# cbouilla/spasm

Hardware: AMD Instinct MI355X
Metric: rows eliminated/sec (sparse Schur complement, mod 42013) (higher is better)
Workload: dtype i32 sums of i16 x i16 products

## Files before the change

spasm_amd/csrc/backsolve.hip:

```cpp
#include <algorithm>
#include <cinttypes>
#include <type_traits>
#include <thread>
#include <vector>

#include "device_types.h"
#include "field_dev.h"
#include "sgn_dev.h"

namespace sh {

int usable_cpus();

namespace {

constexpr int BS_RING = 768;
constexpr int BS_NEARCAP = 1024;
constexpr int BS_PASSCAP = 80;
constexpr int BS_PASSROWS = 32;
constexpr uint32_t BS_NONE = 0xFFFFFFFFu;

template <typename T> T *dalloc(int64_t count)
{
	return static_cast<T *>(sh::big_alloc((size_t) (count > 0 ? count : 1) * sizeof(T)));
}

template <typename T> void upload(T *dst, const std::vector<T> &src, hipStream_t s)
{
	if (!src.empty())
		sh::h2d(dst, src.data(), src.size() * sizeof(T), s);
}

struct BsArgs {
	void *R;
	int64_t ldR;
	int nchunks;
	const BsChunk *chunk;
	const int *chunk_extra;
	const uint4 *ptab;
	const uint2 *near;
	const uint4 *far_head;
	const uint64_t *far_rp;
	const uint2 *far;
	const uint64_t *np_rp;
	const uint2 *np;
	const int *np_row;
	int plain;
	int sparse_init;
	int r;
	unsigned long long *prof;
	int sgn;
	MontDev F;
	SgnDev G;
};

template <bool PACKED> struct Word {
	static constexpr int CPL = PACKED ? 2 : 1;
	using Elem = typename std::conditional<PACKED, uint16_t, uint32_t>::type;
};

template <bool PACKED, bool PLAIN> __device__ __forceinline__ uint32_t w_submul(uint32_t x, uint32_t v, uint32_t y, const MontDev &F, uint32_t bm)
{
	auto small = [&](uint32_t xe, uint32_t ve) -> uint32_t {
		const uint32_t t = __umul24(ve, y);
		const uint32_t q = __umulhi(t, bm);
		uint32_t rem = t - __umul24(q, F.p);
		rem = (rem >= F.p) ? rem - F.p : rem;
		rem = (rem >= F.p) ? rem - F.p : rem;
		return (xe >= rem) ? xe - rem : xe + F.p - rem;
	};
	if constexpr (PACKED) {
		static_assert(PLAIN, "packed entries only exist for p < 2^16");
		return small(x & 0xFFFFu, v & 0xFFFFu) | (small(x >> 16, v >> 16) << 16);
	} else if constexpr (PLAIN) {
		return small(x, v);
	} else {
		return submod(x, montmul(v, y, F), F);
	}
}

template <typename T> __global__ __launch_bounds__(256) void bs_init_kernel(BsArgs b)
{
// ... 38 lines not shown
}

template <int HI, bool FIRST> __device__ __forceinline__ void sgn_mad_half(uint32_t w, uint32_t c2, int &lo, int &hi)
{
	if constexpr (FIRST) {
		static_assert(HI == 0, "the first term takes the low coefficient");
		asm("v_mad_i32_i16 %0, %1, %2, 0" : "=v"(lo) : "v"(w), "v"(c2));
		asm("v_mad_i32_i16 %0, %1, %2, 0 op_sel:[1,0,0,0]" : "=v"(hi) : "v"(w), "v"(c2));
	} else if constexpr (HI == 0) {
		asm("v_mad_i32_i16 %0, %1, %2, %0" : "+v"(lo) : "v"(w), "v"(c2));
		asm("v_mad_i32_i16 %0, %1, %2, %0 op_sel:[1,0,0,0]" : "+v"(hi) : "v"(w), "v"(c2));
	} else {
		asm("v_mad_i32_i16 %0, %1, %2, %0 op_sel:[0,1,0,0]" : "+v"(lo) : "v"(w), "v"(c2));
		asm("v_mad_i32_i16 %0, %1, %2, %0 op_sel:[1,1,0,0]" : "+v"(hi) : "v"(w), "v"(c2));
	}
}

__host__ __device__ __forceinline__ uint4 bs_pass_empty(uint32_t spare_off)
{
	return uint4{spare_off, spare_off | (spare_off << 16), 0u, 0u};
}

template <int HI> __device__ __forceinline__ uint32_t bs_ring_at(uint32_t packed, uint32_t base)
{
	uint32_t a;
	if constexpr (HI == 0)
		asm("v_mad_u32_u16 %0, %1, 4, %2" : "=v"(a) : "v"(packed), "v"(base));
	else
		asm("v_mad_u32_u16 %0, %1, 4, %2 op_sel:[1,0,0,0]" : "=v"(a) : "v"(packed), "v"(base));
	return a;
}
using bs_lds_word = __attribute__((address_space(3))) uint32_t;

template <bool PACKED, int LPR, int NW, int RING = BS_RING, int PASSROWS = BS_PASSROWS, int PASSCAP = BS_PASSCAP> struct BsGeom {
	static constexpr int RING_ = RING, PASSROWS_ = PASSROWS, PASSCAP_ = PASSCAP;
	static constexpr int THREADS = 64 * NW;
	static constexpr int RS = 64 / LPR;
	static constexpr int CW = LPR * Word<PACKED>::CPL;
	static constexpr int ROWS_PER_ITER = RS * NW;
	static constexpr int ITERS = RING / ROWS_PER_ITER;
	static constexpr int UNR = (NW >= 8 && ITERS <= 24) ? ITERS : (ITERS % 12 == 0) ? 12 : 8;
	static constexpr int LANES_USED = RS * LPR;
	static_assert(RING % ROWS_PER_ITER == 0 && ITERS % UNR == 0, "phase A is unrolled in passes of UNR rows");
	static constexpr int N_NEAR = (BS_NEARCAP + THREADS - 1) / THREADS;
	static constexpr int N_ROW = (RING + THREADS - 1) / THREADS;
	static constexpr int N_PTAB = (PASSCAP * PASSROWS + THREADS - 1) / THREADS;
	static constexpr size_t FH_BYTES = (size_t) RING * sizeof(uint4);
	static constexpr size_t PTAB_BYTES = (size_t) PASSCAP * PASSROWS * sizeof(uint4);
	static constexpr int RSTR = LPR + 1;
	static constexpr size_t LDS_BYTES = FH_BYTES + PTAB_BYTES + (size_t) BS_NEARCAP * sizeof(uint2) + (size_t) (RING + 1) * RSTR * 4;
};

template <bool PACKED, bool PLAIN, int LPR, int NW, bool SGN = false, int RING = BS_RING, int PASSROWS = BS_PASSROWS, int PASSCAP = BS_PASSCAP, int WGS_PER_CU = 1>
__global__ __launch_bounds__(64 * NW, WGS_PER_CU) void backsolve_kernel(BsArgs b)
{
	static_assert(!SGN || (PACKED && PLAIN), "signed entries are packed 16-bit entries");
	const uint32_t bm = PLAIN ? (uint32_t) (0x100000000ull / b.F.p) : 0u;
	const SgnDev G = b.G;
	using Geo = BsGeom<PACKED, LPR, NW, RING, PASSROWS, PASSCAP>;
	using Elem = typename Word<PACKED>::Elem;
	extern __shared__ __attribute__((aligned(16))) unsigned char bs_lds[];
	uint4 *fh = reinterpret_cast<uint4 *>(bs_lds);
	uint4 *ptab = reinterpret_cast<uint4 *>(bs_lds + Geo::FH_BYTES);
	uint2 *near = reinterpret_cast<uint2 *>(bs_lds + Geo::FH_BYTES + Geo::PTAB_BYTES);
	uint32_t *ring = reinterpret_cast<uint32_t *>(near + BS_NEARCAP);
	const int tid = threadIdx.x;
	const int lane = tid & 63, wave = tid >> 6;
	auto lds_barrier = [&]() { asm volatile("s_waitcnt lgkmcnt(0)\n\ts_barrier" ::: "memory"); };
	const int rs = lane / LPR, wl = lane % LPR;
	constexpr int RSTR = Geo::RSTR;
	constexpr uint32_t SPARE = (uint32_t) (RING * RSTR);
	constexpr int WPW = LPR / NW, RSB = 64 / WPW;
	static_assert(WPW >= 1 && LPR % NW == 0 && 64 % WPW == 0, "every wave takes the same number of words of a row through phase B");
	static_assert(PASSROWS % RSB == 0, "a pass is a whole number of wave instructions");
	const MontDev F = b.F;
	const int64_t ldw = b.ldR / Word<PACKED>::CPL;
	uint32_t *Rs = static_cast<uint32_t *>(b.R) + (int64_t) blockIdx.x * LPR + wl;
	const uint32_t ldw256 = (uint32_t) (ldw >> 8);
	auto at_off = [&](uint32_t off) -> uint32_t * { return Rs + ((uint64_t) off << 8); };
	const int slot0 = wave * Geo::RS + rs;
	const uint32_t slot0_off = (uint32_t) slot0 * ldw256;
	const uint32_t iter_off = (uint32_t) Geo::ROWS_PER_ITER * ldw256;
	const bool lane_ok = lane < Geo::LANES_USED && (int64_t) blockIdx.x * LPR + wl < ldw;
	const int col_lo = blockIdx.x * Geo::CW;

	RegFile<uint2, Geo::N_NEAR> m_near;
	RegFile<uint4, Geo::N_ROW> m_fh;
	RegFile<uint4, Geo::N_PTAB> m_ptab;
	auto load_meta = [&](const BsChunk &c) {
		bs_static_for<0, Geo::N_NEAR>([&](auto qq) {
			constexpr int q = decltype(qq)::value;
			const int t = tid + q * Geo::THREADS;
			const uint2 v = b.near[(t < c.nnear) ? c.near0 + t : 0];
			m_near.template at<q>() = (t < c.nnear) ? v : uint2{0u, 0u};
		});
		bs_static_for<0, Geo::N_ROW>([&](auto qq) {
			constexpr int q = decltype(qq)::value;
			const int t = tid + q * Geo::THREADS;
			const uint4 v = b.far_head[(t < c.hi - c.lo) ? c.lo + t : 0];
			m_fh.template at<q>() = (t < c.hi - c.lo) ? v : bs_head<PLAIN>(BS_NONE, 0u, BS_NONE, 0u);
		});
		int tid_m = tid;
		asm volatile("" : "+v"(tid_m));
		bs_static_for<0, Geo::N_PTAB>([&](auto qq) {
			constexpr int q = decltype(qq)::value;
			const int t = tid_m + q * Geo::THREADS;
			const uint4 v = b.ptab[(t < c.npass * PASSROWS) ? (int64_t) c.pass0 * PASSROWS + t : 0];
			m_ptab.template at<q>() = (t < c.npass * PASSROWS) ? v : bs_pass_empty(SPARE);
		});
	};
	auto store_meta = [&]() {
		bs_static_for<0, Geo::N_NEAR>([&](auto qq) {
			constexpr int q = decltype(qq)::value;
			if (tid + q * Geo::THREADS < BS_NEARCAP)
				near[tid + q * Geo::THREADS] = m_near.template at<q>();
		});
		bs_static_for<0, Geo::N_ROW>([&](auto qq) {
// ... 12 lines not shown
	asm volatile("v_mov_b32 %0, 0" : "=v"(vzero));
	uint4 raw_a = uint4{0u, 0u, 0u, 0u}, raw_b = uint4{0u, 0u, 0u, 0u};
	auto fetch_chunk = [&](int k) {
		const uint4 *src = reinterpret_cast<const uint4 *>(b.chunk + k) + vzero;
		raw_a = src[0];
		raw_b = src[1];
	};
	auto fetched_chunk = [&]() {
		BsChunk c;
		c.lo = __builtin_amdgcn_readfirstlane((int) raw_a.x);
		c.hi = __builtin_amdgcn_readfirstlane((int) raw_a.y);
		c.pass0 = __builtin_amdgcn_readfirstlane((int) raw_a.z);
		c.npass = (unsigned short) __builtin_amdgcn_readfirstlane((int) (raw_a.w & 0xFFFFu));
		c.nord = (unsigned short) __builtin_amdgcn_readfirstlane((int) (raw_a.w >> 16));
		c.near0 = __builtin_amdgcn_readfirstlane((int) raw_b.x);
		c.nnear = __builtin_amdgcn_readfirstlane((int) raw_b.y);
		c.np0 = __builtin_amdgcn_readfirstlane((int) raw_b.z);
		c.npn = __builtin_amdgcn_readfirstlane((int) raw_b.w);
		return c;
	};
	BsChunk ch_next{};
	if (b.nchunks > 0) {
		fetch_chunk(0);
		ch_next = fetched_chunk();
		load_meta(ch_next);
		store_meta();
	}
	if (b.nchunks > 1)
		fetch_chunk(1);
	__syncthreads();

	unsigned long long pt[8] = {0, 0, 0, 0, 0, 0, 0, 0};
	unsigned long long t_last = 0;
	const bool profiling = b.prof != nullptr && blockIdx.x == 0 && tid == 0;
	auto tick = [&](int q) {
		if (profiling) {
			const unsigned long long now = __builtin_readcyclecounter();
			pt[q] += now - t_last;
			t_last = now;
		}
	};
	if (profiling)
		t_last = __builtin_readcyclecounter();
	for (int k = 0; k < b.nchunks; k++) {
		const BsChunk ch = ch_next;
		const int nrows = ch.hi - ch.lo;
		uint2 c_np = uint2{0u, 0u};
		int c_np_row = 0;
		if (b.sparse_init) {
			const int cnt = ch.npn & 0x7FFFFFFF;
			c_np = b.np[(tid < cnt) ? ch.np0 + tid : 0];
			c_np_row = b.np_row[(tid < cnt) ? ch.np0 + tid : 0];
		}
		if (k + 1 < b.nchunks) {
			ch_next = fetched_chunk();
			load_meta(ch_next);
		}
		if (k + 2 < b.nchunks)
			fetch_chunk(k + 2);
		tick(0);

		const uint32_t lo_off = (uint32_t) ch.lo * ldw256;
		auto phase_a = [&](auto sparse_tag) {
			constexpr bool SPARSE = decltype(sparse_tag)::value;
			for (int pass = 0; pass < Geo::ITERS / Geo::UNR; pass++) {
				if (pass * Geo::UNR * Geo::ROWS_PER_ITER >= nrows)
					break;
				constexpr bool KEEP = SPARSE && (PLAIN || NW < 16);
				uint32_t acc[SPARSE ? 1 : Geo::UNR], v0[Geo::UNR], v1[Geo::UNR], c0[KEEP ? Geo::UNR : 1], c1[(KEEP && !PLAIN) ? Geo::UNR : 1];
				uint32_t own_off = lo_off + (uint32_t) (pass * Geo::UNR) * iter_off + slot0_off;
				asm volatile("" : "+v"(own_off));
#pragma unroll
				for (int u = 0; u < Geo::UNR; u++) {
					const int s = (pass * Geo::UNR + u) * Geo::ROWS_PER_ITER + slot0;
					const bool ok = s < nrows && lane_ok;
					const uint4 h = fh[ok ? s : 0];
					const uint32_t a0 = h.x, a1 = PLAIN ? h.y : h.z;
					if constexpr (KEEP) {
						c0[u] = PLAIN ? h.z : h.y;
						if constexpr (!PLAIN)
							c1[u] = h.w;
					}
					if constexpr (!SPARSE) {
						acc[u] = ok ? *at_off(own_off) : 0u;
						own_off += iter_off;
					}
					if constexpr (LPR <= 16 && 64 % LPR == 0) {
						v0[u] = *at_off((ok && a0 != BS_NONE) ? a0 : lo_off);
						v1[u] = *at_off((ok && a1 != BS_NONE) ? a1 : lo_off);
					} else {
						v0[u] = (ok && a0 != BS_NONE) ? *at_off(a0) : 0u;
						v1[u] = (ok && a1 != BS_NONE) ? *at_off(a1) : 0u;
					}
				}
#pragma unroll
				for (int u = 0; u < Geo::UNR; u++) {
					const int s = (pass * Geo::UNR + u) * Geo::ROWS_PER_ITER + slot0;
					uint32_t x = SPARSE ? 0u : acc[u];
					uint32_t k0, k1;
					if constexpr (KEEP) {
						k0 = c0[u];
						k1 = PLAIN ? 0u : c1[u];
					} else if constexpr (PLAIN) {
						k0 = fh[s].z;
						k1 = 0u;
					} else {
						const uint4 h = fh[s];
						k0 = h.y;
						k1 = h.w;
					}
					if constexpr (SGN) {
						int lo, hi;
						if constexpr (SPARSE) {
							sgn_mad_half<0, true>(v0[u], k0, lo, hi);
						} else {
							sgn_unpack(x, lo, hi);
							sgn_mad_half<0, false>(v0[u], k0, lo, hi);
						}
						sgn_mad_half<1, false>(v1[u], k0, lo, hi);
						x = sgn_pack(sgn_reduce(lo, G), sgn_reduce(hi, G));
					} else {
						if constexpr (PLAIN) {
							k1 = k0 >> 16;
							k0 &= 0xFFFFu;
						}
						if (k0 != 0u)
							x = w_submul<PACKED, PLAIN>(x, v0[u], k0, F, bm);
						if (k1 != 0u)
							x = w_submul<PACKED, PLAIN>(x, v1[u], k1, F, bm);
					}
					if (s < nrows && lane_ok)
						ring[s * RSTR + wl] = x;
				}
			}
		};
		if (b.sparse_init)
			phase_a(std::true_type{});
		else
			phase_a(std::false_type{});
		lds_barrier();
		tick(1);
		if (b.sparse_init) {
			const int np_count = ch.npn & 0x7FFFFFFF;
			auto put = [&](const uint2 en, int row) {
				const int cc = (int) en.x - col_lo;
				if (cc >= 0 && cc < Geo::CW) {
					Elem *at = reinterpret_cast<Elem *>(ring) + (row - ch.lo) * (RSTR * Word<PACKED>::CPL) + cc;
					if constexpr (SGN) {
						*at = (Elem) (uint16_t) (int16_t) sgn_canonical((int) (int16_t) *at + sgn_from_residue(en.y, G), G);
					} else {
						const uint32_t v = PLAIN ? en.y : montmul(en.y, 1u, F);
						uint32_t sum = (uint32_t) *at + v;
						if (sum < v || sum >= F.p)
							sum -= F.p;
						*at = (Elem) sum;
					}
				}
			};
			if (tid < np_count)
				put(c_np, c_np_row);
			for (int e = Geo::THREADS + tid; e < np_count; e += Geo::THREADS)
				put(b.np[ch.np0 + e], b.np_row[ch.np0 + e]);
			lds_barrier();
		}
		tick(2);
		if (ch.npn < 0) {
			for (int s = slot0; s < nrows; s += Geo::ROWS_PER_ITER) {
				const int c = ch.lo + s;
				const uint64_t e0 = b.far_rp[c], e1 = b.far_rp[c + 1];
				if (e0 == e1 || !lane_ok)
					continue;
				uint32_t x = ring[s * RSTR + wl];
				if constexpr (SGN) {
					int lo, hi;
					sgn_unpack(x, lo, hi);
					for (uint64_t e = e0; e < e1; e += 4) {
#pragma unroll
						for (int t = 0; t < 4; t++) {
							const uint2 en = (e + t < e1) ? b.far[e + t] : uint2{0u, 0u};
							sgn_mad((e + t < e1) ? *at_off(en.x) : 0u, (int) en.y, lo, hi);
						}
						lo = sgn_reduce(lo, G);
						hi = sgn_reduce(hi, G);
					}
					x = sgn_pack(lo, hi);
				} else {
					for (uint64_t e = e0; e < e1; e++) {
						const uint2 en = b.far[e];
						x = w_submul<PACKED, PLAIN>(x, *at_off(en.x), en.y, F, bm);
					}
				}
				ring[s * RSTR + wl] = x;
			}
			lds_barrier();
		}

		tick(3);
		{
			constexpr int IPP = PASSROWS / RSB;
			const int niter = ch.npass * IPP;
			int tid_b = tid;
			asm volatile("" : "+v"(tid_b));
			const int rsb = (tid_b & 63) / WPW, wlb = (tid_b >> 6) * WPW + (tid_b & 63) % WPW;
			const uint4 *pe = ptab + rsb;
			const uint32_t wlb_at = (uint32_t) (uintptr_t) (bs_lds_word *) (ring + wlb);
			auto word = [&](uint32_t at) -> bs_lds_word & { return *reinterpret_cast<bs_lds_word *>((uintptr_t) at); };
			auto ordinary = [&](const uint4 e) {
				const uint32_t at_x = bs_ring_at<0>(e.x, wlb_at), at_0 = bs_ring_at<0>(e.y, wlb_at), at_1 = bs_ring_at<1>(e.y, wlb_at);
				if constexpr (SGN) {
					const uint32_t x0 = word(at_x), v0 = word(at_0), v1 = word(at_1);
					int lo, hi;
					sgn_unpack(x0, lo, hi);
					sgn_mad_half<0, false>(v0, e.z, lo, hi);
					sgn_mad_half<1, false>(v1, e.z, lo, hi);
					word(at_x) = sgn_pack(sgn_reduce(lo, G), sgn_reduce(hi, G));
				} else {
					const uint32_t c0 = PLAIN ? (e.z & 0xFFFFu) : e.z, c1 = PLAIN ? (e.z >> 16) : e.w;
					if (c0 != 0u) {
						uint32_t x = w_submul<PACKED, PLAIN>(word(at_x), word(at_0), c0, F, bm);
						if (c1 != 0u)
							x = w_submul<PACKED, PLAIN>(x, word(at_1), c1, F, bm);
						word(at_x) = x;
					}
				}
			};
// ... 33 lines not shown
			uint4 e = pe[0];
			int it = 0, run = ch.nord * IPP;
			while (it < niter) {
				const int stop = min(it + run, niter);
				for (; it + 1 < stop; it += 2) {
					const uint4 e_odd = pe[(it + 1) * RSB];
					ordinary(e);
					e = pe[(it + 2) * RSB];
					ordinary(e_odd);
				}
				if (it < stop) {
					const uint4 e_next = pe[(it + 1) * RSB];
					ordinary(e);
					e = e_next;
					it += 1;
				}
				if (it < niter) {
					run = __builtin_amdgcn_readfirstlane((int) (e.y >> 16)) * IPP;
					for (int q = 0; q < IPP; q++, it++) {
						const uint4 e_next = pe[(it + 1) * RSB];
						long_row(e);
						e = e_next;
					}
				}
			}
		}
		lds_barrier();
		tick(4);

		{
			uint32_t off = lo_off + slot0_off;
			asm volatile("" : "+v"(off));
			for (int s = slot0; s < nrows; s += Geo::ROWS_PER_ITER, off += iter_off)
				if (lane_ok)
					*at_off(off) = ring[s * RSTR + wl];
		}
		__syncthreads();
		tick(5);
		if (k + 1 < b.nchunks)
			store_meta();
		__syncthreads();
		tick(6);
	}
	if (profiling)
		for (int q = 0; q < 8; q++)
			b.prof[q] = pt[q];
}

constexpr int AP_LIST = 64;
constexpr int AP_TU = 4;

struct ApplyArgs {
	SchurArgs a;
	const void *R;
	int64_t ldR;
	const int *col;
	int r;
	int Smpad;
	int seg_words;
	int waves;
	size_t wave_bytes;
	uint32_t *dense_out;
	int64_t ldS;
	int direct;
	unsigned long long *status;
	int *ticket;
	int ntickets;
	int64_t *Sp;
	int *Sj;
	int *Sx;
// ... 252 lines not shown
						out_x[wpos + before] = to_balanced(v0, F);
					}
					if (v1 != 0) {
						const int64_t dst = wpos + before + (v0 != 0 ? 1 : 0);
						out_j[dst] = a.q[c0 + 1];
						out_x[dst] = to_balanced(v1, F);
					}
					wpos += __popcll(m0) + __popcll(m1);
				} else {
					const uint64_t mk = __ballot(w != 0);
					if (w != 0) {
						const int64_t dst = wpos + __popcll(mk & below);
						out_j[dst] = a.q[t0 + lane];
						out_x[dst] = to_balanced(w, F);
					}
					wpos += __popcll(mk);
				}
			}
		}
		if (lane == 0 && !d.direct) {
			if (fits) {
				a.row_off[k] = off | (1LL << 62);
				a.row_len[k] = count;
			} else {
				atomicOr(&a.ctr[CTR_STATUS], 1);
				a.row_len[k] = -1;
			}
		}
		st_done += fits ? 1 : 0;
	}
	apply_statistics(a, lane, st_input, st_piv, st_done, lost);
}

template <bool DEEP>
__device__ __forceinline__ int s16_reduce_segment(const ApplyArgs &d, const MontDev &F, const SgnDev &G, int64_t lo, int64_t hi, int w0, int nwords,
                                                  uint2 *plist, uint32_t *xw, int lane, bool first_seg, unsigned long long &st_piv)
{
	short *xe = reinterpret_cast<short *>(xw);
	const uint32_t *R = static_cast<const uint32_t *>(d.R);
	const uint32_t ldw256 = (uint32_t) (d.ldR / 2 / 256);
	for (int t = lane; t < nwords; t += 64)
		xw[t] = 0;
	int npl = 0;
	int count = -1;
	for (int64_t base = lo;; base += 64) {
		bool piv = false;
		uint32_t cid = 0;
		int bal = 0;
		if (base + lane < hi) {
			cid = (uint32_t) d.col[d.a.Aj[base + lane]];
			bal = sgn_from_residue(reduce_sum(from_balanced(d.a.Ax[base + lane], F), F), G);
			if (cid >= (uint32_t) d.r) {
				const uint32_t t = cid - (uint32_t) d.r - 2u * (uint32_t) w0;
				if (t < 2u * (uint32_t) nwords)
					xe[t] = (short) sgn_canonical((int) xe[t] + bal, G);
			} else {
				piv = bal != 0;
			}
		}
		const uint64_t mk = __ballot(piv);
		if (piv)
			plist[npl + __popcll(mk & ((1ull << lane) - 1ull))] = uint2{cid * ldw256, (uint32_t) (-bal)};
		npl += __popcll(mk);
		st_piv += first_seg ? (unsigned long long) __popcll(mk) : 0ull;
		const bool last = base + 64 >= hi;
		if (npl > 0 && (last || npl + 64 > AP_LIST)) {
			const int ne = (npl + 3) >> 2;
			const int nunits = (nwords / (64 * AP_TU)) * ne;
			int cnt = 0;
			int alo[AP_TU], ahi[AP_TU];
			uint32_t wa[4][AP_TU], wb[4][AP_TU], wc[4][AP_TU];
			int ca[4], cb[4], cc[4];
			int pf_t0 = 0, pf_e = 0;
			const int t0_last = nwords - 64 * AP_TU;
			const int64_t row_mask = (d.dbg & 8) ? 0 : -1;
			auto issue = [&](uint32_t (&w)[4][AP_TU], int (&cf)[4]) {
				const int t0c = (pf_t0 < t0_last) ? pf_t0 : t0_last;
#pragma unroll
				for (int q = 0; q < 4; q++) {
					const int idx = (pf_e + q < npl) ? pf_e + q : npl - 1;
					const uint2 pe = plist[idx];
					cf[q] = (pf_e + q < npl) ? (int) pe.y : 0;
					const uint32_t *rq = R + ((((uint64_t) pe.x) << 8) & (uint64_t) row_mask) + w0 + t0c + lane;
#pragma unroll
					for (int u = 0; u < AP_TU; u++)
						w[q][u] = rq[u * 64];
				}
				pf_e += 4;
				const bool wrap = pf_e >= npl;
				pf_e = wrap ? 0 : pf_e;
				pf_t0 += wrap ? 64 * AP_TU : 0;
			};
			int t0 = 0, e = 0;
// ... 160 lines not shown
				uint32_t dst = wpos;
				dst = __builtin_amdgcn_mbcnt_hi((uint32_t) (m0 >> 32), __builtin_amdgcn_mbcnt_lo((uint32_t) m0, dst));
				dst = __builtin_amdgcn_mbcnt_hi((uint32_t) (m1 >> 32), __builtin_amdgcn_mbcnt_lo((uint32_t) m1, dst));
				if (v0 != 0) {
					oj[dst] = qq.x;
					ox[dst] = v0;
					dst += 1;
				}
				if (v1 != 0) {
					oj[dst] = qq.y;
					ox[dst] = v1;
				}
				wpos += (uint32_t) (__popcll(m0) + __popcll(m1));
			}
		}
		if (lane == 0 && !d.direct) {
			if (fits) {
				a.row_off[k] = off | (1LL << 62);
				a.row_len[k] = count;
			} else {
				atomicOr(&a.ctr[CTR_STATUS], 1);
				a.row_len[k] = -1;
			}
		}
		st_done += fits ? 1 : 0;
	  }
	}
	apply_statistics(a, lane, st_input, st_piv, st_done, lost);
}

constexpr int CSR_SCRATCH_BYTES = 512 * 4;
static_assert(CSR_SCRATCH_BYTES >= AP_LIST * (int) sizeof(uint2), "the list shares the compaction area");

template <typename WordAt>
__device__ __forceinline__ void csr_emit_group(WordAt &&word, const int2 (&qq)[AP_TU], const SgnDev &G, int *cbuf, int *oj, int *ox, uint32_t &wpos, int lane)
{
	int v0[AP_TU], v1[AP_TU];
	uint32_t dst[AP_TU], gpos = 0;
	bs_static_for<0, AP_TU>([&](auto uu) {
		constexpr int u = decltype(uu)::value;
		sgn_unpack(word(uu), v0[u], v1[u]);
		v0[u] = sgn_canonical(v0[u], G);
		v1[u] = sgn_canonical(v1[u], G);
		const uint64_t m0 = __ballot(v0[u] != 0), m1 = __ballot(v1[u] != 0);
		uint32_t at = gpos;
		at = __builtin_amdgcn_mbcnt_hi((uint32_t) (m0 >> 32), __builtin_amdgcn_mbcnt_lo((uint32_t) m0, at));
		at = __builtin_amdgcn_mbcnt_hi((uint32_t) (m1 >> 32), __builtin_amdgcn_mbcnt_lo((uint32_t) m1, at));
		dst[u] = at;
		if (v0[u] != 0)
			cbuf[at] = qq[u].x;
		if (v1[u] != 0)
			cbuf[at + (v0[u] != 0 ? 1u : 0u)] = qq[u].y;
		gpos += (uint32_t) (__popcll(m0) + __popcll(m1));
	});
	for (uint32_t t = lane; t < gpos; t += 64)
		oj[wpos + t] = cbuf[t];
#pragma unroll
	for (int u = 0; u < AP_TU; u++) {
		if (v0[u] != 0)
			cbuf[dst[u]] = v0[u];
		if (v1[u] != 0)
			cbuf[dst[u] + (v0[u] != 0 ? 1u : 0u)] = v1[u];
	}
	for (uint32_t t = lane; t < gpos; t += 64)
		ox[wpos + t] = cbuf[t];
	wpos += gpos;
}

template <bool DEEP>
__device__ __forceinline__ int csr_produce_row(const ApplyArgs &d, const MontDev &F, const SgnDev &G, int nwords, uint2 *plist, uint32_t *xw, int lane,
                                               int &count, unsigned long long &st_input, unsigned long long &st_piv)
{
	const int k = next_ticket(d, lane);
	if (k >= d.a.nrows)
		return k;
	const int i = d.a.rows[k];
	const int64_t lo = d.a.Ap[i], hi = d.a.Ap[i + 1];
	st_input += (unsigned long long) (hi - lo);
	count = s16_reduce_segment<DEEP>(d, F, G, lo, hi, 0, nwords, plist, xw, lane, true, st_piv);
	if (count < 0)
		count = s16_count_entries(xw, nwords, lane);
	lb_publish_length(d, k, count, lane);
	return k;
}

struct PendingLds {
	int nwords;
	uint32_t *xc, *xp;

	__device__ __forceinline__ PendingLds(const ApplyArgs &d, uint32_t *rows) : nwords(d.Smpad / 2), xc(rows), xp(rows + d.Smpad / 2) {}

	__device__ __forceinline__ void hand_over(int)
	{
		uint32_t *const t = xp;
		xp = xc;
		xc = t;
	}

// ... 414 lines not shown
			}
			const int word = w0 + u * 64 + lane;
			if constexpr (PACKED) {
				if (2 * word < a.Sm)
					out[2 * word] = lo_s;
				if (2 * word + 1 < a.Sm)
					out[2 * word + 1] = hi_s;
			} else {
				if (word < a.Sm)
					out[word] = lo_s;
			}
		}
		if (lane == 0 && blockIdx.x == 0) {
			a.row_len[k] = a.Sm;
			atomicAdd(&a.ctr[a.done_ctr], 1);
			atomicAdd(&a.ctr64[C64_INPUT], (unsigned long long) (hi - lo));
		}
	}
}

template <bool PACKED, bool PLAIN, int LPR, int NW, bool SGN = false, int RING = BS_RING, int PASSROWS = BS_PASSROWS, int PASSCAP = BS_PASSCAP, int WGS_PER_CU = 1>
void launch_backsolve_variant(const BsArgs &b, int Sm, hipStream_t stream, const BsImage &B)
{
	using G = BsGeom<PACKED, LPR, NW, RING, PASSROWS, PASSCAP>;
	if (B.ring != RING || B.passrows != PASSROWS || B.passcap != PASSCAP || B.rstr != G::RSTR)
		die("backsolve: the plan was built for chunks of %d rows, passes of %d rows, %d passes, ring rows %d words apart; this kernel takes %d / %d / %d / %d",
		    B.ring, B.passrows, B.passcap, B.rstr, RING, PASSROWS, PASSCAP, G::RSTR);
	static bool configured = false;
	if (!configured) {
		HIP_CHECK(hipFuncSetAttribute(reinterpret_cast<const void *>(&backsolve_kernel<PACKED, PLAIN, LPR, NW, SGN, RING, PASSROWS, PASSCAP, WGS_PER_CU>),
		                              hipFuncAttributeMaxDynamicSharedMemorySize, (int) G::LDS_BYTES));
		configured = true;
	}
	hipLaunchKernelGGL((backsolve_kernel<PACKED, PLAIN, LPR, NW, SGN, RING, PASSROWS, PASSCAP, WGS_PER_CU>), dim3((unsigned) ((Sm + G::CW - 1) / G::CW)),
	                   dim3(64 * NW), G::LDS_BYTES, stream, b);
}

template <bool PACKED, bool PLAIN> void launch_apply_variant(const ApplyArgs &d, int blocks, size_t lds, hipStream_t stream)
{
	static size_t configured = 0;
	if (lds > configured) {
		HIP_CHECK(hipFuncSetAttribute(reinterpret_cast<const void *>(&bs_apply_kernel<PACKED, PLAIN>),
		                              hipFuncAttributeMaxDynamicSharedMemorySize, (int) lds));
		configured = lds;
	}
	hipLaunchKernelGGL((bs_apply_kernel<PACKED, PLAIN>), dim3(blocks), dim3(64 * d.waves), lds, stream, d);
}

}

void launch_scan_lengths(const int *len, int n, const unsigned long long *block_sum, int64_t *Sp, int64_t cap, int *ctr, hipStream_t stream)
{
	if (n <= 0)
		return;
	hipLaunchKernelGGL(bs_scan_lengths_kernel, dim3((n + SCAN_BLOCK - 1) / SCAN_BLOCK), dim3(SCAN_BLOCK), 0, stream, len, n, block_sum, Sp, cap, ctr);
}

bool backsolve_eligible(int r, int Sm, int64_t nnz_u, int64_t *bytes, int64_t prime)
{
	const int64_t ldR = ((int64_t) Sm + 511) / 512 * 512;
	*bytes = (int64_t) r * ldR * 4;
	if (r <= 0 || Sm <= 0)
		return false;
	const bool segments = prime < 65536 && sgn_eligible(prime) && env_int("SPASM_HIP_BS_SIGNED", 1) != 0 &&
	                      env_int("SPASM_HIP_BS_STAGED", 1) != 0;
	if (Sm > (segments ? 131072 : 24576))
		return false;
	if ((double) (nnz_u + r) * (double) Sm > 1.5e11)
// ... 412 lines not shown
		die("backsolve_build: the factor has no back-substitution plan");
	const bool packed = F->prime < 65536;
	const int elem = packed ? 2 : 4;
	const size_t bytes = (size_t) B.r * (size_t) B.ldR * (size_t) elem;
	if (B.d_R != nullptr && B.elem_bytes != elem) {
		big_free(B.d_R);
		B.d_R = nullptr;
	}
	bool fresh = false;
	if (B.d_R == nullptr) {
		B.d_R = big_alloc(bytes);
		B.elem_bytes = elem;
		fresh = true;
	}
	if (B.ev0 == nullptr) {
		HIP_CHECK(hipEventCreate(&B.ev0));
		HIP_CHECK(hipEventCreate(&B.ev1));
	}
	BsArgs b{};
	b.R = B.d_R;
	b.ldR = B.ldR;
	b.nchunks = B.nchunks;
	b.chunk = B.d_chunk;
	b.chunk_extra = B.d_chunk_extra;
	b.ptab = B.d_ptab;
	b.near = B.d_near;
	b.far_head = B.d_far_head;
	b.far_rp = B.d_far_rp;
	b.far = B.d_far;
	b.np_rp = B.d_np_rp;
	b.np = B.d_np;
	b.np_row = B.d_np_row;
	b.r = B.r;
	b.plain = B.plain ? 1 : 0;
	b.sgn = B.sgn ? 1 : 0;
	b.G = sgn_setup(F->prime);
	b.F = to_dev(F->mont);
	b.prof = nullptr;
	if (env_int("SPASM_HIP_BS_PROFILE", 0)) {
		b.prof = dalloc<unsigned long long>(8);
		HIP_CHECK(hipMemsetAsync(b.prof, 0, 8 * sizeof(unsigned long long), stream));
	}
	b.sparse_init = (B.nnp <= 4 * (int64_t) B.r && env_int("SPASM_HIP_BS_SPARSE_INIT", 1) != 0) ? 1 : 0;
	HIP_CHECK(hipEventRecord(B.ev0, stream));
	if (fresh || !b.sparse_init)
		HIP_CHECK(hipMemsetAsync(B.d_R, 0, bytes, stream));
	if (!b.sparse_init) {
		if (packed)
			hipLaunchKernelGGL(bs_init_kernel<uint16_t>, dim3((B.r + 255) / 256), dim3(256), 0, stream, b);
		else
			hipLaunchKernelGGL(bs_init_kernel<uint32_t>, dim3((B.r + 255) / 256), dim3(256), 0, stream, b);
	}
	const int shape = B.shape;
	if (shape == 3)
		snprintf(B.kernel_build, sizeof(B.kernel_build), "backsolve_kernel<true,true,8,8,true,768,64,31,2>");
	else if (shape == 4)
		snprintf(B.kernel_build, sizeof(B.kernel_build), "backsolve_kernel<true,true,10,10,true,1260,64,48,1>");
	else if (shape == 5)
		snprintf(B.kernel_build, sizeof(B.kernel_build), "backsolve_kernel<true,true,12,12,true,1200,64,44,1>");
	else
		snprintf(B.kernel_build, sizeof(B.kernel_build), "backsolve_kernel<%s,%s,%d,%d,%s,%d,%d,%d,1>", packed ? "true" : "false", B.plain ? "true" : "false",
		         shape == 2 ? 16 : 32, (shape == 0 || (!packed && B.plain && shape == 1)) ? 16 : 8, B.sgn ? "true" : "false", BS_RING, BS_PASSROWS,
		         BS_PASSCAP);
	if (B.sgn) {
		if (shape == 3)
			launch_backsolve_variant<true, true, 8, 8, true, 768, 64, 31, 2>(b, B.Sm, stream, B);
// ... 5 lines not shown
			launch_backsolve_variant<true, true, 32, 8, true>(b, B.Sm, stream, B);
		else if (shape == 2)
			launch_backsolve_variant<true, true, 16, 8, true>(b, B.Sm, stream, B);
		else
			launch_backsolve_variant<true, true, 32, 16, true>(b, B.Sm, stream, B);
	} else if (packed) {
		if (shape == 1)
			launch_backsolve_variant<true, true, 32, 8>(b, B.Sm, stream, B);
		else if (shape == 2)
			launch_backsolve_variant<true, true, 16, 8>(b, B.Sm, stream, B);
		else
			launch_backsolve_variant<true, true, 32, 16>(b, B.Sm, stream, B);
	} else if (B.plain) {
		if (shape == 2)
			launch_backsolve_variant<false, true, 16, 8>(b, B.Sm, stream, B);
		else
			launch_backsolve_variant<false, true, 32, 16>(b, B.Sm, stream, B);
	} else {
		if (shape == 1)
			launch_backsolve_variant<false, false, 32, 8>(b, B.Sm, stream, B);
		else if (shape == 2)
			launch_backsolve_variant<false, false, 16, 8>(b, B.Sm, stream, B);
		else
			launch_backsolve_variant<false, false, 32, 16>(b, B.Sm, stream, B);
	}
	HIP_CHECK(hipGetLastError());
	HIP_CHECK(hipEventRecord(B.ev1, stream));
	B.valid = true;
	B.builds += 1;
	if (b.prof != nullptr) {
		unsigned long long h[8];
		HIP_CHECK(hipMemcpyAsync(h, b.prof, sizeof(h), hipMemcpyDeviceToHost, stream));
		HIP_CHECK(hipStreamSynchronize(stream));
		static const char *const stage[7] = {"descriptor + metadata issue", "phase A", "non-pivotal entries added", "long outside lists", "phase B", "phase C",
		                                     "metadata into LDS"};
		unsigned long long tot = 0;
		for (int q = 0; q < 7; q++)
			tot += h[q];
		fprintf(stderr, "[bs profile] %s, %d chunks, workgroup 0, shader-clock cycles per chunk:", B.kernel_build, B.nchunks);
		for (int q = 0; q < 7; q++)
			fprintf(stderr, " %s %.0f (%.0f%%);", stage[q], (double) h[q] / B.nchunks, 100.0 * (double) h[q] / (double) (tot ? tot : 1));
		fprintf(stderr, " total %.0f\n", (double) tot / B.nchunks);
		sh::big_free(b.prof);
	}
}

bool backsolve_stages_output(const spasm_hip_dfact *F, int64_t *row_bytes)
{
	const BsImage &B = F->bs;
	*row_bytes = B.ldR * (B.valid ? B.elem_bytes : 4);
	return B.planned && env_int("SPASM_HIP_BS_STAGED", 1) != 0;
}

static size_t csr_wave_bytes(int64_t ldR, int buffers)
{
	return (size_t) CSR_SCRATCH_BYTES + (size_t) buffers * (size_t) ldR * 2;
}

static int csr_rowreg_tiles(int64_t ldR)
{
	if (ldR > 128 * CSR_ROWREG_MAX_TILES || env_int("SPASM_HIP_BS_CSR_ROWREG", 1) == 0)
		return 0;
	return (int) (ldR / 128);
}

using CsrKernel = void (*)(ApplyArgs);
static CsrKernel csr_kernel(int tiles)
{
// ... 178 lines not shown
```

Measured before the change: 38.71 million.

## Add short-row fast path for few pivots and buffer-store CSR copy-out

Rows that fit in a single 64-entry batch and have at most four pivot terms now skip zeroing the dense row and the pivot-list machinery. A specialized routine reads up to four pivot rows with scalar coefficients, accumulates them using packed i16 mad instructions, and writes the reduced row directly. The non-pivot entries are applied afterwards while the nonzero count is adjusted incrementally. The CSR emit loop also replaces per-lane bounded stores with unconditional raw buffer stores whose bounds come from the buffer descriptor, removing loop control in exchange for inline asm and fixed copy passes.

After: 39.42 million, median of 6. 1.8% higher.

```diff
diff --git a/spasm_amd/csrc/backsolve.hip b/spasm_amd/csrc/backsolve.hip
--- a/spasm_amd/csrc/backsolve.hip
+++ b/spasm_amd/csrc/backsolve.hip
@@ -861,6 +861,84 @@
 	apply_statistics(a, lane, st_input, st_piv, st_done, lost);
 }
 
+
+template <bool FIRST> __device__ __forceinline__ void sgn_mad_uniform(uint32_t w, int c, int &lo, int &hi)
+{
+	if constexpr (FIRST) {
+		asm("v_mad_i32_i16 %0, %1, %2, 0" : "=v"(lo) : "v"(w), "s"(c));
+		asm("v_mad_i32_i16 %0, %1, %2, 0 op_sel:[1,0,0,0]" : "=v"(hi) : "v"(w), "s"(c));
+	} else {
+		asm("v_mad_i32_i16 %0, %1, %2, %0" : "+v"(lo) : "v"(w), "s"(c));
+		asm("v_mad_i32_i16 %0, %1, %2, %0 op_sel:[1,0,0,0]" : "+v"(hi) : "v"(w), "s"(c));
+	}
+}
+
+template <int Q>
+__device__ __forceinline__ int s16_reduce_short(const ApplyArgs &d, const SgnDev &G, int w0, int nwords, uint32_t *xw, int lane, uint64_t pivots, uint32_t cid,
+                                                int bal, bool nonpiv, uint32_t t)
+{
+	static_assert(Q >= 1 && Q <= 4, "one reduction after at most four terms");
+	constexpr int GW = 64 * AP_TU;
+	const uint32_t ldw256 = (uint32_t) (d.ldR / 2 / 256);
+	const uint32_t *row[Q];
+	int cf[Q];
+#pragma unroll
+	for (int q = 0; q < Q; q++) {
+		const int from = __builtin_ctzll(pivots);
+		pivots &= pivots - 1ull;
+		row[q] = static_cast<const uint32_t *>(d.R) + (((uint64_t) ((uint32_t) __builtin_amdgcn_readlane((int) cid, from) * ldw256)) << 8) + w0;
+		cf[q] = -__builtin_amdgcn_readlane(bal, from);
+	}
+	uint32_t wa[Q][AP_TU], wb[Q][AP_TU];
+	const int t0_last = nwords - GW;
+	auto issue = [&](int t0, uint32_t (&w)[Q][AP_TU]) {
+		const uint32_t at = (uint32_t) ((t0 < t0_last ? t0 : t0_last) + lane);
+#pragma unroll
+		for (int q = 0; q < Q; q++) {
+			const uint32_t *rq = row[q] + at;
+#pragma unroll
+			for (int u = 0; u < AP_TU; u++)
+				w[q][u] = rq[u * 64];
+		}
+	};
+	int cnt = 0;
+	auto multiply = [&](int t0, const uint32_t (&w)[Q][AP_TU]) {
+#pragma unroll
+		for (int u = 0; u < AP_TU; u++) {
+			int al, ah;
+			sgn_mad_uniform<true>(w[0][u], cf[0], al, ah);
+#pragma unroll
+			for (int q = 1; q < Q; q++)
+				sgn_mad_uniform<false>(w[q][u], cf[q], al, ah);
+			const int rl = sgn_reduce(al, G), rh = sgn_reduce(ah, G);
+			xw[t0 + u * 64 + lane] = sgn_pack(rl, rh);
+			cnt += __popcll(__ballot(rl != 0)) + __popcll(__ballot(rh != 0));
+		}
+	};
+	issue(0, wa);
+	for (int t0 = 0; t0 < nwords; t0 += 2 * GW) {
+		issue(t0 + GW, wb);
+		multiply(t0, wa);
+		issue(t0 + 2 * GW, wa);
+		if (t0 + GW < nwords)
+			multiply(t0 + GW, wb);
+	}
+	if (__ballot(nonpiv) != 0) {
+		__builtin_amdgcn_fence(__ATOMIC_ACQ_REL, "wavefront");
+		short *xe = reinterpret_cast<short *>(xw);
+		bool was = false, is = false;
+		if (nonpiv) {
+			const int before = (int) xe[t];
+			const int after = sgn_canonical(before + bal, G);
+			xe[t] = (short) after;
+			was = before != 0;
+			is = after != 0;
+		}
+		cnt += __popcll(__ballot(is)) - __popcll(__ballot(was));
+	}
+	return cnt;
+}
+
 template <bool DEEP>
 __device__ __forceinline__ int s16_reduce_segment(const ApplyArgs &d, const MontDev &F, const SgnDev &G, int64_t lo, int64_t hi, int w0, int nwords,
                                                   uint2 *plist, uint32_t *xw, int lane, bool first_seg, unsigned long long &st_piv)
@@ -868,26 +946,45 @@
 	short *xe = reinterpret_cast<short *>(xw);
 	const uint32_t *R = static_cast<const uint32_t *>(d.R);
 	const uint32_t ldw256 = (uint32_t) (d.ldR / 2 / 256);
-	for (int t = lane; t < nwords; t += 64)
-		xw[t] = 0;
+	auto zero_row = [&]() {
+		for (int t = lane; t < nwords; t += 64)
+			xw[t] = 0;
+	};
+	const bool one_batch = hi - lo <= 64;
+	if (!one_batch)
+		zero_row();
 	int npl = 0;
 	int count = -1;
 	for (int64_t base = lo;; base += 64) {
-		bool piv = false;
-		uint32_t cid = 0;
+		bool piv = false, nonpiv = false;
+		uint32_t cid = 0, t = 0;
 		int bal = 0;
 		if (base + lane < hi) {
 			cid = (uint32_t) d.col[d.a.Aj[base + lane]];
 			bal = sgn_from_residue(reduce_sum(from_balanced(d.a.Ax[base + lane], F), F), G);
 			if (cid >= (uint32_t) d.r) {
-				const uint32_t t = cid - (uint32_t) d.r - 2u * (uint32_t) w0;
-				if (t < 2u * (uint32_t) nwords)
-					xe[t] = (short) sgn_canonical((int) xe[t] + bal, G);
+				t = cid - (uint32_t) d.r - 2u * (uint32_t) w0;
+				nonpiv = t < 2u * (uint32_t) nwords;
 			} else {
 				piv = bal != 0;
 			}
 		}
 		const uint64_t mk = __ballot(piv);
+		if (one_batch) {
+			const int nq = __popcll(mk);
+			if (nq >= 1 && nq <= 4) {
+				st_piv += first_seg ? (unsigned long long) nq : 0ull;
+				switch (nq) {
+				case 1: return s16_reduce_short<1>(d, G, w0, nwords, xw, lane, mk, cid, bal, nonpiv, t);
+				case 2: return s16_reduce_short<2>(d, G, w0, nwords, xw, lane, mk, cid, bal, nonpiv, t);
+				case 3: return s16_reduce_short<3>(d, G, w0, nwords, xw, lane, mk, cid, bal, nonpiv, t);
+				default: return s16_reduce_short<4>(d, G, w0, nwords, xw, lane, mk, cid, bal, nonpiv, t);
+				}
+			}
+			zero_row();
+		}
+		if (nonpiv)
+			xe[t] = (short) sgn_canonical((int) xe[t] + bal, G);
 		if (piv)
 			plist[npl + __popcll(mk & ((1ull << lane) - 1ull))] = uint2{cid * ldw256, (uint32_t) (-bal)};
 		npl += __popcll(mk);
@@ -1114,6 +1211,31 @@
 constexpr int CSR_SCRATCH_BYTES = 512 * 4;
 static_assert(CSR_SCRATCH_BYTES >= AP_LIST * (int) sizeof(uint2), "the list shares the compaction area");
 
+constexpr int CSR_COPY_PASSES = 2 * AP_TU, CSR_COPY_BATCH = 2;
+static_assert(CSR_COPY_PASSES * 64 * (int) sizeof(int) == CSR_SCRATCH_BYTES && CSR_COPY_PASSES % CSR_COPY_BATCH == 0, "the whole area, in whole batches");
+constexpr int BUFFER_RSRC_RAW_DWORDS = 0x00020000;
+
+__device__ __forceinline__ void csr_copy_out(const int *cbuf, int *out, uint32_t n, int lane)
+{
+	const uint64_t at = reinterpret_cast<uint64_t>(out);
+	const uint32_t at_lo = (uint32_t) __builtin_amdgcn_readfirstlane((int) (uint32_t) at);
+	const uint32_t at_hi = (uint32_t) __builtin_amdgcn_readfirstlane((int) (uint32_t) (at >> 32));
+	int *const base = reinterpret_cast<int *>(((uint64_t) at_hi << 32) | (uint64_t) at_lo);
+	const __amdgpu_buffer_rsrc_t rows = __builtin_amdgcn_make_buffer_rsrc(base, 0, (int) (n * (uint32_t) sizeof(int)), BUFFER_RSRC_RAW_DWORDS);
+	int mine = lane * (int) sizeof(int);
+	asm volatile("" : "+v"(mine));
+#pragma unroll
+	for (int b = 0; b < CSR_COPY_PASSES; b += CSR_COPY_BATCH) {
+		int c[CSR_COPY_BATCH];
+#pragma unroll
+		for (int i = 0; i < CSR_COPY_BATCH; i++)
+			c[i] = cbuf[64 * (b + i) + lane];
+#pragma unroll
+		for (int i = 0; i < CSR_COPY_BATCH; i++)
+			__builtin_amdgcn_raw_buffer_store_b32((uint32_t) c[i], rows, mine + 64 * (b + i) * (int) sizeof(int), 0, 0);
+	}
+}
+
 template <typename WordAt>
 __device__ __forceinline__ void csr_emit_group(WordAt &&word, const int2 (&qq)[AP_TU], const SgnDev &G, int *cbuf, int *oj, int *ox, uint32_t &wpos, int lane)
 {
@@ -1135,8 +1257,7 @@
 			cbuf[at + (v0[u] != 0 ? 1u : 0u)] = qq[u].y;
 		gpos += (uint32_t) (__popcll(m0) + __popcll(m1));
 	});
-	for (uint32_t t = lane; t < gpos; t += 64)
-		oj[wpos + t] = cbuf[t];
+	csr_copy_out(cbuf, oj + wpos, gpos, lane);
 #pragma unroll
 	for (int u = 0; u < AP_TU; u++) {
 		if (v0[u] != 0)
@@ -1144,8 +1265,7 @@
 		if (v1[u] != 0)
 			cbuf[dst[u] + (v0[u] != 0 ? 1u : 0u)] = v1[u];
 	}
-	for (uint32_t t = lane; t < gpos; t += 64)
-		ox[wpos + t] = cbuf[t];
+	csr_copy_out(cbuf, ox + wpos, gpos, lane);
 	wpos += gpos;
 }
 
```

## Vectorize backsolve row words, remap workgroups across XCDs, drop trailing barrier

Applied to the files above, without the earlier changes.

When the wave count equals lanes-per-row, each lane now moves four consecutive words with 128-bit loads and stores in phase A and the write-back, so fewer lanes cover a row and more rows fit per wave instruction. Workgroup indices are permuted so that adjacent column slabs land on the same XCD, with padding blocks exiting early. The outside-list loop keeps the one-word-per-lane mapping. The __syncthreads after phase C write-back is removed, leaving only the barrier in the metadata stage to order chunks, which risks a race if that barrier is not enough.

Result: faster. 40.62 million before, 43.43 million after (median of 6 runs) (+6.9%).

```diff
diff --git a/spasm_amd/csrc/backsolve.hip b/spasm_amd/csrc/backsolve.hip
--- a/spasm_amd/csrc/backsolve.hip
+++ b/spasm_amd/csrc/backsolve.hip
@@ -19,6 +19,7 @@
 constexpr int BS_PASSCAP = 80;
 constexpr int BS_PASSROWS = 32;
 constexpr uint32_t BS_NONE = 0xFFFFFFFFu;
+constexpr int BS_XCDS = 8;
 
 template <typename T> T *dalloc(int64_t count)
 {
@@ -48,6 +49,7 @@
 	int plain;
 	int sparse_init;
 	int r;
+	int Sm;
 	unsigned long long *prof;
 	int sgn;
 	MontDev F;
@@ -152,15 +154,42 @@
 }
 using bs_lds_word = __attribute__((address_space(3))) uint32_t;
 
+template <int WPL> __device__ __forceinline__ void bs_load_words(bool present, const uint32_t *at, uint32_t (&w)[WPL])
+{
+	static_assert(WPL == 1 || WPL == 4, "a lane moves one word or four");
+	if constexpr (WPL == 4) {
+		const uint4 t = present ? *reinterpret_cast<const uint4 *>(at) : uint4{0u, 0u, 0u, 0u};
+		w[0] = t.x, w[1] = t.y, w[2] = t.z, w[3] = t.w;
+	} else {
+		w[0] = present ? *at : 0u;
+	}
+}
+template <int WPL> __device__ __forceinline__ void bs_store_words(uint32_t *at, const uint32_t (&w)[WPL])
+{
+	if constexpr (WPL == 4)
+		*reinterpret_cast<uint4 *>(at) = uint4{w[0], w[1], w[2], w[3]};
+	else
+		*at = w[0];
+}
+
+constexpr int bs_rows_dividing(int rows, int nw, int ring)
+{
+	return (rows <= 1 || ring % (rows * nw) == 0) ? rows : bs_rows_dividing(rows - 1, nw, ring);
+}
+
 template <bool PACKED, int LPR, int NW, int RING = BS_RING, int PASSROWS = BS_PASSROWS, int PASSCAP = BS_PASSCAP> struct BsGeom {
 	static constexpr int RING_ = RING, PASSROWS_ = PASSROWS, PASSCAP_ = PASSCAP;
 	static constexpr int THREADS = 64 * NW;
-	static constexpr int RS = 64 / LPR;
+	static constexpr int WPL = (NW == LPR && LPR % 4 == 0) ? 4 : 1;
+	static constexpr int QPR = LPR / WPL;
+	static constexpr int RS = (WPL == 1) ? 64 / QPR : bs_rows_dividing(64 / QPR, NW, RING);
+	static constexpr int RS1 = 64 / LPR;
 	static constexpr int CW = LPR * Word<PACKED>::CPL;
 	static constexpr int ROWS_PER_ITER = RS * NW;
 	static constexpr int ITERS = RING / ROWS_PER_ITER;
 	static constexpr int UNR = (NW >= 8 && ITERS <= 24) ? ITERS : (ITERS % 12 == 0) ? 12 : 8;
-	static constexpr int LANES_USED = RS * LPR;
+	static constexpr int LANES_USED = RS * QPR;
+	static_assert(LPR % WPL == 0 && LANES_USED <= 64, "a row is whole lanes, a wave instruction whole rows");
 	static_assert(RING % ROWS_PER_ITER == 0 && ITERS % UNR == 0, "phase A is unrolled in passes of UNR rows");
 	static constexpr int N_NEAR = (BS_NEARCAP + THREADS - 1) / THREADS;
 	static constexpr int N_ROW = (RING + THREADS - 1) / THREADS;
@@ -175,6 +204,10 @@
 __global__ __launch_bounds__(64 * NW, WGS_PER_CU) void backsolve_kernel(BsArgs b)
 {
 	static_assert(!SGN || (PACKED && PLAIN), "signed entries are packed 16-bit entries");
+	const int nslabs = (b.Sm + LPR * Word<PACKED>::CPL - 1) / (LPR * Word<PACKED>::CPL);
+	const int slab = (int) (blockIdx.x % BS_XCDS) * (int) (gridDim.x / BS_XCDS) + (int) (blockIdx.x / BS_XCDS);
+	if (slab >= nslabs)
+		return;
 	const uint32_t bm = PLAIN ? (uint32_t) (0x100000000ull / b.F.p) : 0u;
 	const SgnDev G = b.G;
 	using Geo = BsGeom<PACKED, LPR, NW, RING, PASSROWS, PASSCAP>;
@@ -187,7 +220,8 @@
 	const int tid = threadIdx.x;
 	const int lane = tid & 63, wave = tid >> 6;
 	auto lds_barrier = [&]() { asm volatile("s_waitcnt lgkmcnt(0)\n\ts_barrier" ::: "memory"); };
-	const int rs = lane / LPR, wl = lane % LPR;
+	constexpr int WPL = Geo::WPL;
+	const int rs = lane / Geo::QPR, wl = lane % Geo::QPR * WPL;
 	constexpr int RSTR = Geo::RSTR;
 	constexpr uint32_t SPARE = (uint32_t) (RING * RSTR);
 	constexpr int WPW = LPR / NW, RSB = 64 / WPW;
@@ -195,14 +229,15 @@
 	static_assert(PASSROWS % RSB == 0, "a pass is a whole number of wave instructions");
 	const MontDev F = b.F;
 	const int64_t ldw = b.ldR / Word<PACKED>::CPL;
-	uint32_t *Rs = static_cast<uint32_t *>(b.R) + (int64_t) blockIdx.x * LPR + wl;
+	uint32_t *Rs = static_cast<uint32_t *>(b.R) + (int64_t) slab * LPR + wl;
 	const uint32_t ldw256 = (uint32_t) (ldw >> 8);
 	auto at_off = [&](uint32_t off) -> uint32_t * { return Rs + ((uint64_t) off << 8); };
 	const int slot0 = wave * Geo::RS + rs;
 	const uint32_t slot0_off = (uint32_t) slot0 * ldw256;
 	const uint32_t iter_off = (uint32_t) Geo::ROWS_PER_ITER * ldw256;
-	const bool lane_ok = lane < Geo::LANES_USED && (int64_t) blockIdx.x * LPR + wl < ldw;
-	const int col_lo = blockIdx.x * Geo::CW;
+	static_assert(WPL == 1 || (LPR % WPL == 0 && 256 % WPL == 0), "WPL words at a multiple of WPL: one aligned access, inside the padded row or outside it");
+	const bool lane_ok = lane < Geo::LANES_USED && (int64_t) slab * LPR + wl < ldw;
+	const int col_lo = slab * Geo::CW;
 
 	RegFile<uint2, Geo::N_NEAR> m_near;
 	RegFile<uint4, Geo::N_ROW> m_fh;
@@ -281,7 +316,7 @@
 
 	unsigned long long pt[8] = {0, 0, 0, 0, 0, 0, 0, 0};
 	unsigned long long t_last = 0;
-	const bool profiling = b.prof != nullptr && blockIdx.x == 0 && tid == 0;
+	const bool profiling = b.prof != nullptr && slab == 0 && tid == 0;
 	auto tick = [&](int q) {
 		if (profiling) {
 			const unsigned long long now = __builtin_readcyclecounter();
@@ -316,7 +351,7 @@
 				if (pass * Geo::UNR * Geo::ROWS_PER_ITER >= nrows)
 					break;
 				constexpr bool KEEP = SPARSE && (PLAIN || NW < 16);
-				uint32_t acc[SPARSE ? 1 : Geo::UNR], v0[Geo::UNR], v1[Geo::UNR], c0[KEEP ? Geo::UNR : 1], c1[(KEEP && !PLAIN) ? Geo::UNR : 1];
+				uint32_t acc[SPARSE ? 1 : Geo::UNR][WPL], v0[Geo::UNR][WPL], v1[Geo::UNR][WPL], c0[KEEP ? Geo::UNR : 1], c1[(KEEP && !PLAIN) ? Geo::UNR : 1];
 				uint32_t own_off = lo_off + (uint32_t) (pass * Geo::UNR) * iter_off + slot0_off;
 				asm volatile("" : "+v"(own_off));
 #pragma unroll
@@ -331,21 +366,20 @@
 							c1[u] = h.w;
 					}
 					if constexpr (!SPARSE) {
-						acc[u] = ok ? *at_off(own_off) : 0u;
+						bs_load_words<WPL>(ok, at_off(own_off), acc[u]);
 						own_off += iter_off;
 					}
 					if constexpr (LPR <= 16 && 64 % LPR == 0) {
-						v0[u] = *at_off((ok && a0 != BS_NONE) ? a0 : lo_off);
-						v1[u] = *at_off((ok && a1 != BS_NONE) ? a1 : lo_off);
+						bs_load_words<WPL>(true, at_off((ok && a0 != BS_NONE) ? a0 : lo_off), v0[u]);
+						bs_load_words<WPL>(true, at_off((ok && a1 != BS_NONE) ? a1 : lo_off), v1[u]);
 					} else {
-						v0[u] = (ok && a0 != BS_NONE) ? *at_off(a0) : 0u;
-						v1[u] = (ok && a1 != BS_NONE) ? *at_off(a1) : 0u;
+						bs_load_words<WPL>(ok && a0 != BS_NONE, at_off(a0), v0[u]);
+						bs_load_words<WPL>(ok && a1 != BS_NONE, at_off(a1), v1[u]);
 					}
 				}
 #pragma unroll
 				for (int u = 0; u < Geo::UNR; u++) {
 					const int s = (pass * Geo::UNR + u) * Geo::ROWS_PER_ITER + slot0;
-					uint32_t x = SPARSE ? 0u : acc[u];
 					uint32_t k0, k1;
 					if constexpr (KEEP) {
 						k0 = c0[u];
@@ -358,28 +392,33 @@
 						k0 = h.y;
 						k1 = h.w;
 					}
-					if constexpr (SGN) {
-						int lo, hi;
-						if constexpr (SPARSE) {
-							sgn_mad_half<0, true>(v0[u], k0, lo, hi);
+					uint32_t x[WPL];
+#pragma unroll
+					for (int j = 0; j < WPL; j++) {
+						x[j] = SPARSE ? 0u : acc[u][j];
+						if constexpr (SGN) {
+							int lo, hi;
+							if constexpr (SPARSE) {
+								sgn_mad_half<0, true>(v0[u][j], k0, lo, hi);
+							} else {
+								sgn_unpack(x[j], lo, hi);
+								sgn_mad_half<0, false>(v0[u][j], k0, lo, hi);
+							}
+							sgn_mad_half<1, false>(v1[u][j], k0, lo, hi);
+							x[j] = sgn_pack(sgn_reduce(lo, G), sgn_reduce(hi, G));
 						} else {
-							sgn_unpack(x, lo, hi);
-							sgn_mad_half<0, false>(v0[u], k0, lo, hi);
+							const uint32_t q0 = PLAIN ? (k0 & 0xFFFFu) : k0, q1 = PLAIN ? (k0 >> 16) : k1;
+							if (q0 != 0u)
+								x[j] = w_submul<PACKED, PLAIN>(x[j], v0[u][j], q0, F, bm);
+							if (q1 != 0u)
+								x[j] = w_submul<PACKED, PLAIN>(x[j], v1[u][j], q1, F, bm);
 						}
-						sgn_mad_half<1, false>(v1[u], k0, lo, hi);
-						x = sgn_pack(sgn_reduce(lo, G), sgn_reduce(hi, G));
-					} else {
-						if constexpr (PLAIN) {
-							k1 = k0 >> 16;
-							k0 &= 0xFFFFu;
-						}
-						if (k0 != 0u)
-							x = w_submul<PACKED, PLAIN>(x, v0[u], k0, F, bm);
-						if (k1 != 0u)
-							x = w_submul<PACKED, PLAIN>(x, v1[u], k1, F, bm);
 					}
-					if (s < nrows && lane_ok)
-						ring[s * RSTR + wl] = x;
+					if (s < nrows && lane_ok) {
+#pragma unroll
+						for (int j = 0; j < WPL; j++)
+							ring[s * RSTR + wl + j] = x[j];
+					}
 				}
 			}
 		};
@@ -414,12 +453,24 @@
 		}
 		tick(2);
 		if (ch.npn < 0) {
-			for (int s = slot0; s < nrows; s += Geo::ROWS_PER_ITER) {
+			int slot1 = slot0, wl1 = wl;
+			bool ok1 = lane_ok;
+			const uint32_t *R1 = Rs;
+			if constexpr (WPL > 1) {
+				int tid_l = tid;
+				asm volatile("" : "+v"(tid_l));
+				wl1 = (tid_l & 63) % LPR;
+				slot1 = (tid_l >> 6) * Geo::RS1 + (tid_l & 63) / LPR;
+				ok1 = (tid_l & 63) < Geo::RS1 * LPR && (int64_t) slab * LPR + wl1 < ldw;
+				R1 = static_cast<const uint32_t *>(b.R) + (int64_t) slab * LPR + wl1;
+			}
+			auto at_off1 = [&](uint32_t off) -> const uint32_t * { return R1 + ((uint64_t) off << 8); };
+			for (int s = slot1; s < nrows; s += Geo::RS1 * NW) {
 				const int c = ch.lo + s;
 				const uint64_t e0 = b.far_rp[c], e1 = b.far_rp[c + 1];
-				if (e0 == e1 || !lane_ok)
+				if (e0 == e1 || !ok1)
 					continue;
-				uint32_t x = ring[s * RSTR + wl];
+				uint32_t x = ring[s * RSTR + wl1];
 				if constexpr (SGN) {
 					int lo, hi;
 					sgn_unpack(x, lo, hi);
@@ -427,7 +478,7 @@
 #pragma unroll
 						for (int t = 0; t < 4; t++) {
 							const uint2 en = (e + t < e1) ? b.far[e + t] : uint2{0u, 0u};
-							sgn_mad((e + t < e1) ? *at_off(en.x) : 0u, (int) en.y, lo, hi);
+							sgn_mad((e + t < e1) ? *at_off1(en.x) : 0u, (int) en.y, lo, hi);
 						}
 						lo = sgn_reduce(lo, G);
 						hi = sgn_reduce(hi, G);
@@ -436,10 +487,10 @@
 				} else {
 					for (uint64_t e = e0; e < e1; e++) {
 						const uint2 en = b.far[e];
-						x = w_submul<PACKED, PLAIN>(x, *at_off(en.x), en.y, F, bm);
+						x = w_submul<PACKED, PLAIN>(x, *at_off1(en.x), en.y, F, bm);
 					}
 				}
-				ring[s * RSTR + wl] = x;
+				ring[s * RSTR + wl1] = x;
 			}
 			lds_barrier();
 		}
@@ -539,10 +590,14 @@
 			uint32_t off = lo_off + slot0_off;
 			asm volatile("" : "+v"(off));
 			for (int s = slot0; s < nrows; s += Geo::ROWS_PER_ITER, off += iter_off)
-				if (lane_ok)
-					*at_off(off) = ring[s * RSTR + wl];
-		}
-		__syncthreads();
+				if (lane_ok) {
+					uint32_t x[WPL];
+#pragma unroll
+					for (int j = 0; j < WPL; j++)
+						x[j] = ring[s * RSTR + wl + j];
+					bs_store_words<WPL>(at_off(off), x);
+				}
+		}
 		tick(5);
 		if (k + 1 < b.nchunks)
 			store_meta();
@@ -1626,8 +1681,9 @@
 		                              hipFuncAttributeMaxDynamicSharedMemorySize, (int) G::LDS_BYTES));
 		configured = true;
 	}
-	hipLaunchKernelGGL((backsolve_kernel<PACKED, PLAIN, LPR, NW, SGN, RING, PASSROWS, PASSCAP, WGS_PER_CU>), dim3((unsigned) ((Sm + G::CW - 1) / G::CW)),
-	                   dim3(64 * NW), G::LDS_BYTES, stream, b);
+	const int nslabs = (Sm + G::CW - 1) / G::CW;
+	hipLaunchKernelGGL((backsolve_kernel<PACKED, PLAIN, LPR, NW, SGN, RING, PASSROWS, PASSCAP, WGS_PER_CU>),
+	                   dim3((unsigned) ((nslabs + BS_XCDS - 1) / BS_XCDS * BS_XCDS)), dim3(64 * NW), G::LDS_BYTES, stream, b);
 }
 
 template <bool PACKED, bool PLAIN> void launch_apply_variant(const ApplyArgs &d, int blocks, size_t lds, hipStream_t stream)
@@ -2106,6 +2162,7 @@
 	b.np = B.d_np;
 	b.np_row = B.d_np_row;
 	b.r = B.r;
+	b.Sm = B.Sm;
 	b.plain = B.plain ? 1 : 0;
 	b.sgn = B.sgn ? 1 : 0;
 	b.G = sgn_setup(F->prime);
@@ -2177,8 +2234,8 @@
 		unsigned long long h[8];
 		HIP_CHECK(hipMemcpyAsync(h, b.prof, sizeof(h), hipMemcpyDeviceToHost, stream));
 		HIP_CHECK(hipStreamSynchronize(stream));
-		static const char *const stage[7] = {"descriptor + metadata issue", "phase A", "non-pivotal entries added", "long outside lists", "phase B", "phase C",
-		                                     "metadata into LDS"};
+		static const char *const stage[7] = {"descriptor + metadata issue", "phase A", "non-pivotal entries added", "long outside lists", "phase B", "phase C (issue)",
+		                                     "metadata into LDS + barrier"};
 		unsigned long long tot = 0;
 		for (int q = 0; q < 7; q++)
 			tot += h[q];
```
